# drnatebrown/col-bwt

Measured on AMD Instinct MI355X. Metric: query bases/s, higher is better.
Workload: dtype int64

## Files before the change

col-bwt_amd/csrc/capi.hip:

```cpp
#include <fcntl.h>
#include <hip/hip_runtime.h>
#include <stdlib.h>
#include <string.h>
#include <sys/mman.h>
#include <sys/stat.h>
#include <unistd.h>

#include <algorithm>
#include <atomic>
#include <chrono>
#include <condition_variable>
#include <deque>
#include <mutex>
#include <string>
#include <thread>
#include <vector>

#include "../../include/colbwt.h"
#include "bin_writer.h"
#include "count_query.h"
#include "fasta_parallel.h"
#include "fastx_reader.h"
#include "index.h"
#include "locate_query.h"
// ... 757 lines not shown
    if (e && e[0] >= '1' && e[0] <= '6' && e[1] == 0) return e[0] - '0';
    return COLBWT_LAYOUT_DEFAULT_CHOICE;
}

static int line_rows_steps(int layout_arg) {
    int steps = (layout_arg >> 8) & 0xFF;
    if (steps == 0) {
        steps = kDefaultLineSteps;
        const char *e = getenv("COLBWT_LINE_ROWS_STEPS");
        if (e && e[0] >= '2' && e[0] <= '8' && e[1] == 0) steps = e[0] - '0';
    }
    return steps;
}

int colbwt_index_open_memory(const void *bytes, uint64_t len, const colbwt_widths *widths, int device,
                             colbwt_index **out) {
    return colbwt_index_open_memory_layout(bytes, len, widths, device, COLBWT_LAYOUT_AUTO, out);
}

int colbwt_index_open_memory_layout(const void *bytes, uint64_t len, const colbwt_widths *widths, int device,
                                    int layout, colbwt_index **out) {
    if (!out) return fail(COLBWT_ERR_ARG, "null out");
    const bool automatic = layout == COLBWT_LAYOUT_AUTO;
    if (automatic) layout = default_layout();
    const int steps = line_rows_steps(layout);
    const bool steps_given = ((layout >> 8) & 0xFF) != 0 || getenv("COLBWT_LINE_ROWS_STEPS") != nullptr;
    layout &= 0xFF;
    if (layout < COLBWT_LAYOUT_ONE_STEP || layout > COLBWT_LAYOUT_MISMATCH_LINES_DEEP) return fail(COLBWT_ERR_ARG, "bad layout");
    if (layout >= COLBWT_LAYOUT_LINE_ROWS && !fat_steps_supported(steps))
        return fail(COLBWT_ERR_ARG, "line rows: own steps must be 4..8");
    *out = nullptr;
    if (!widths_ok(widths))
        return fail(COLBWT_ERR_ARG, "only the shipped widths BWT_BYTES=5 RUN_BYTES=4 LEN_BYTES=2 ID_BITS=8 are supported");
    colbwt_index *idx = new (std::nothrow) colbwt_index();
    if (!idx) return fail(COLBWT_ERR_NOMEM, "out of host memory");
    std::string err;
    const bool deep_if_room = automatic && layout == COLBWT_LAYOUT_MISMATCH_LINES && getenv("COLBWT_LAYOUT") == nullptr;
    int rc = idx->ix.load((const uint8_t *)bytes, len, device, deep_if_room ? kLayoutMismatchLinesAuto : layout, err, steps);
    if (rc == COLBWT_ERR_NOMEM && automatic) {
        struct Candidate { int layout, steps; };
        static const Candidate ladder[] = {{COLBWT_LAYOUT_MISMATCH_LINES_DEEP, 8}, {COLBWT_LAYOUT_MISMATCH_LINES, 8},
                                           {COLBWT_LAYOUT_LINE_ROWS, 8}, {COLBWT_LAYOUT_LINE_ROWS, 6},
                                           {COLBWT_LAYOUT_LINE_ROWS, 4},      {COLBWT_LAYOUT_THREE_STEP, 0}, {COLBWT_LAYOUT_TWO_STEP, 0},
                                           {COLBWT_LAYOUT_ONE_STEP, 0}};
        int hopeless_from = layout >= COLBWT_LAYOUT_LINE_ROWS ? idx->ix.fat_failed_level() : 0;
        for (const Candidate &c : ladder) {
            if (c.layout > layout || (c.layout == layout && (c.steps >= steps || steps_given))) continue;
            if (c.layout >= COLBWT_LAYOUT_LINE_ROWS && (steps_given || (hopeless_from && c.steps >= hopeless_from))) continue;
            rc = idx->ix.load((const uint8_t *)bytes, len, device, c.layout, err, c.steps);
            if (rc != COLBWT_ERR_NOMEM) break;
            if (c.layout >= COLBWT_LAYOUT_LINE_ROWS) {
                const int f = idx->ix.fat_failed_level();
                if (f && (!hopeless_from || f < hopeless_from)) hopeless_from = f;
            }
        }
    }
    if (rc != COLBWT_OK) {
        delete idx;
        return fail(rc, err);
    }
    *out = idx;
    return COLBWT_OK;
}

int colbwt_index_open(const char *prefix_or_file, const colbwt_widths *widths, int device, colbwt_index **out) {
    return colbwt_index_open_layout(prefix_or_file, widths, device, COLBWT_LAYOUT_AUTO, out);
}

int colbwt_index_open_layout(const char *prefix_or_file, const colbwt_widths *widths, int device, int layout,
                             colbwt_index **out) {
    if (!prefix_or_file || !out) return fail(COLBWT_ERR_ARG, "null argument");
    *out = nullptr;
    MappedFile mf;
    const int rc = map_index_file(prefix_or_file, mf);
    return rc != COLBWT_OK ? rc : colbwt_index_open_memory_layout(mf.data, mf.len, widths, device, layout, out);
}

int colbwt_index_open_memory_devices(const void *bytes, uint64_t len, const colbwt_widths *widths, const int *devices,
                                     int n_devices, int layout, colbwt_index **out) {
    if (!out) return fail(COLBWT_ERR_ARG, "null out");
    *out = nullptr;
    if (!devices || n_devices < 1 || n_devices > 64) return fail(COLBWT_ERR_ARG, "device list must hold 1 .. 64 devices");
    colbwt_index *first = nullptr;
    int rc = colbwt_index_open_memory_layout(bytes, len, widths, devices[0], layout, &first);
    if (rc != COLBWT_OK) return rc;
    colbwt_info info;
    (void)colbwt_index_info(first, &info);
    const int same = (int)info.layout | (info.layout >= COLBWT_LAYOUT_LINE_ROWS ? (int)(info.layout_shape >> 8) << 8 : 0);
    for (int k = 1; k < n_devices; ++k) {
        colbwt_index *rep = nullptr;
        rc = colbwt_index_open_memory_layout(bytes, len, widths, devices[k], same, &rep);
        if (rc != COLBWT_OK) {
            const std::string msg = "replica on device " + std::to_string(devices[k]) + ": " + g_err;
            delete first;
            return fail(rc, msg);
        }
        first->more.push_back(rep);
    }
    *out = first;
    return COLBWT_OK;
}

int colbwt_index_open_devices(const char *prefix_or_file, const colbwt_widths *widths, const int *devices, int n_devices,
                              int layout, colbwt_index **out) {
    if (!prefix_or_file || !out) return fail(COLBWT_ERR_ARG, "null argument");
    *out = nullptr;
    MappedFile mf;
    const int rc = map_index_file(prefix_or_file, mf);
    return rc != COLBWT_OK ? rc : colbwt_index_open_memory_devices(mf.data, mf.len, widths, devices, n_devices, layout, out);
}

void colbwt_index_close(colbwt_index *idx) { delete idx; }

int colbwt_index_info(const colbwt_index *idx, colbwt_info *out) {
    if (!idx || !out) return fail(COLBWT_ERR_ARG, "null argument");
    out->bwt_r = idx->ix.bwt_r();
    out->n = idx->ix.n();
    out->r = idx->ix.r();
    out->sigma = idx->ix.sigma();
    out->device = (uint32_t)idx->ix.device();
    out->device_bytes = idx->ix.device_bytes() + idx->loc.bytes();
    out->layout = (uint32_t)idx->ix.layout();
    out->layout_shape = idx->ix.line_rows() ? (idx->ix.table_fat().steps << 8) | kFatSlotSteps : 0;
    out->table_rows = idx->ix.table_rows();
    out->n_devices = 1 + (uint32_t)idx->more.size();
    out->reserved_ = 0;
    return COLBWT_OK;
}

int colbwt_query_batch(colbwt_index *idx, const uint8_t *bases, const uint64_t *read_off, uint64_t n_reads,
                       uint16_t *pml, uint8_t *cid, colbwt_stats *stats) {
    return query_batch_all<uint16_t>(idx, bases, read_off, n_reads, pml, cid, stats);
}

int colbwt_query_batch_u32(colbwt_index *idx, const uint8_t *bases, const uint64_t *read_off, uint64_t n_reads,
                           uint32_t *pml, uint8_t *cid, colbwt_stats *stats) {
    return query_batch_all<uint32_t>(idx, bases, read_off, n_reads, pml, cid, stats);
}

int colbwt_query_device(colbwt_index *idx, const uint8_t *d_bases, const uint64_t *d_read_off, uint64_t n_reads,
                        uint64_t n_bases, void *d_pml, int pml_bytes, uint8_t *d_cid, void *hip_stream,
                        colbwt_stats *stats) {
    return colbwt_query_device_ordered(idx, d_bases, d_read_off, n_reads, n_bases, d_pml, pml_bytes, d_cid, nullptr,
                                       hip_stream, stats);
}

int colbwt_query_device_ordered(colbwt_index *idx, const uint8_t *d_bases, const uint64_t *d_read_off,
                                uint64_t n_reads, uint64_t n_bases, void *d_pml, int pml_bytes, uint8_t *d_cid,
                                const uint32_t *d_order, void *hip_stream, colbwt_stats *stats) {
    auto bad_argument = [&]() -> const char * {
        if (pml_bytes != 2 && pml_bytes != 4) return "pml_bytes must be 2 or 4";
        if (n_reads == 0) return nullptr;
        if (!d_bases || !d_read_off || !d_pml || !d_cid) return "null device pointer";
        if (((uintptr_t)d_bases & 15) || ((uintptr_t)d_pml & 31) || ((uintptr_t)d_cid & 15))
            return "d_bases/d_cid must be 16-byte aligned and d_pml 32-byte aligned";
        return nullptr;
    };
    return device_entry(idx, d_bases, n_reads, n_bases, hip_stream, kAlgBytesPerBase, stats, bad_argument,
                        [&](const Index &ix, hipStream_t stream) {
                            launch_query(ix, d_bases, d_read_off, n_reads, n_bases, d_pml, pml_bytes, d_cid, d_order, stream);
                        });
}

static int query_file_impl(colbwt_index *idx, const char *pattern_path, const std::string &pml_name,
                           const std::string &cid_name, uint64_t batch_bases, colbwt_stats *stats, bool binary,
                           bool count = false, uint32_t locate_k = 0, uint32_t seeds_min = 0, uint32_t seeds_k = 0) {
    if (stats) memset(stats, 0, sizeof(*stats));
    const size_t replicas = 1 + idx->more.size();
    if (batch_bases == 0) batch_bases = (64ull << 20) * replicas;
    ParallelFasta fasta;
    FastxReader reader;
    bool parallel = fasta.open(pattern_path);
    if (!parallel && !reader.open(pattern_path)) return fail(COLBWT_ERR_IO, std::string("cannot open pattern file ") + pattern_path);
    TextWriter wp, wc;
    BinWriter bp, bc;
    FILE *wn = nullptr;
    if (count) {
        wn = fopen(pml_name.c_str(), "wb");
        if (!wn) return fail(COLBWT_ERR_IO, "cannot create " + pml_name);
        setvbuf(wn, nullptr, _IOFBF, 4u << 20);
    } else {
        if (!(binary ? bp.open(pml_name) : wp.open(pml_name))) return fail(COLBWT_ERR_IO, "cannot create " + pml_name);
        if (!(binary ? bc.open(cid_name) : wc.open(cid_name))) return fail(COLBWT_ERR_IO, "cannot create " + cid_name);
    }
    bool count_ok = true;

    FileBatch pool[kFileBatches];
    std::unique_lock<std::mutex> pinned(idx->file_mu, std::defer_lock);
    if (pinned.try_lock())
        for (int k = 0; k < kFileBatches; ++k) {
            pool[k].pml = &idx->file_pml[k];
            pool[k].cid = &idx->file_cid[k];
        }
    BatchQueue free_q, parsed_q, done_q;
    for (auto &b : pool) free_q.push(&b);
    std::atomic<bool> stop{false};
    std::atomic<bool> reader_failed{false};
    const bool trace = getenv("COLBWT_TRACE") != nullptr;
    double t_parse = 0, t_gpu = 0, t_format = 0;
    auto now = [] { return std::chrono::duration<double>(std::chrono::steady_clock::now().time_since_epoch()).count(); };
    const double t_begin = now();
    const unsigned host_threads = std::min(16u, std::max(2u, std::thread::hardware_concurrency()));

    std::thread reader_thread([&] {
        bool more = true;
        while (more && !stop.load()) {
            FileBatch *b = free_q.pop();
            const double t0 = now();
            b->bases.clear();
            b->names.clear();
            b->off.assign(1, 0);
            uint64_t max_len = 0;
            if (parallel) {
                const ParallelFasta::Result r = fasta.next_batch(batch_bases, host_threads / 2, b->names, b->bases, b->off, max_len);
                if (r == ParallelFasta::kEnd) more = false;
                if (r == ParallelFasta::kNotPlainFasta) {
                    parallel = false;
                    if (!reader.open_at(pattern_path, fasta.position())) {
                        reader_failed.store(true);
                        more = false;
                    }
                }
            }
            if (!parallel && more) {
                std::string name;
                while (b->bases.size() < batch_bases) {
                    if (!reader.next(name, b->bases)) {
                        more = false;
                        break;
                    }
                    b->names.push_back(name);
                    max_len = std::max<uint64_t>(max_len, b->bases.size() - b->off.back());
                    b->off.push_back(b->bases.size());
                }
            }
            b->wide = max_len > 65535;
            t_parse += now() - t0;
            if (b->names.empty()) {
                free_q.push(b);
                if (more) continue;
                break;
            }
            parsed_q.push(b);
        }
        parsed_q.push(nullptr);
    });

    std::thread writer_thread([&] {
        for (;;) {
            FileBatch *b = done_q.pop();
            if (!b) break;
            const uint64_t n_reads = b->names.size();
            const double t0 = now();
            if (seeds_k) {
                const uint32_t *sm = b->pml->as<uint32_t>();
                const uint32_t *sp = b->cid->as<uint32_t>(), *sl = sp + n_reads * seeds_k;
                const uint8_t *sc = (const uint8_t *)(sl + n_reads * seeds_k);
                for (uint64_t k = 0; k < n_reads && count_ok; ++k) {
                    const uint32_t *q = sm + 8 * k;
                    count_ok = fprintf(wn, "%s\t%llu\t%u\t%u\t%u\t%u\t%u\t%u\t%u\t%u\t", b->names[k].c_str(),
                                       (unsigned long long)(b->off[k + 1] - b->off[k]), q[0], q[2], q[1], q[3], q[4], q[5], q[6],
                                       q[7]) > 0;
                    const uint64_t want = std::min<uint64_t>(q[0], seeds_k);
                    for (uint64_t t = 0; t < want && count_ok; ++t) {
                        const uint64_t at = k * seeds_k + t;
                        count_ok = fprintf(wn, t ? ",%u:%u:%u" : "%u:%u:%u", sp[at], sl[at], (unsigned)sc[at]) > 0;
                    }
                    count_ok = count_ok && fputc('\n', wn) != EOF;
                }
                t_format += now() - t0;
                free_q.push(b);
                continue;
            }
            if (count) {
                const uint32_t *ml = b->pml->as<uint32_t>();
                const uint64_t *oc = b->cid->as<uint64_t>();
                const uint64_t *ps = oc + n_reads;
                const std::vector<uint64_t> &ds = idx->loc.doc_start;
                for (uint64_t k = 0; k < n_reads && count_ok; ++k) {
                    count_ok = fprintf(wn, locate_k ? "%s\t%llu\t%u\t%llu\t" : "%s\t%llu\t%u\t%llu\n", b->names[k].c_str(),
                                       (unsigned long long)(b->off[k + 1] - b->off[k]), ml[k], (unsigned long long)oc[k]) > 0;
                    if (!locate_k) continue;
                    const uint64_t want = std::min<uint64_t>(oc[k], locate_k);
                    for (uint64_t t = 0; t < want && count_ok; ++t) {
                        const uint64_t x = ps[k * locate_k + t];
                        const size_t d = (size_t)(std::upper_bound(ds.begin(), ds.end(), x) - ds.begin()) - 1;
                        count_ok = fprintf(wn, t ? ",%zu:%llu" : "%zu:%llu", d, (unsigned long long)(x - ds[d])) > 0;
                    }
                    count_ok = count_ok && fputc('\n', wn) != EOF;
                }
                t_format += now() - t0;
                free_q.push(b);
                continue;
            }
            std::thread cid_thread([&] {
                if (binary) bc.batch<uint8_t>(b->names, b->off.data(), b->cid->as<uint8_t>(), n_reads, host_threads / 2);
                else wc.batch(b->names, b->off.data(), b->cid->as<uint8_t>(), n_reads, host_threads / 2);
            });
            if (binary) {
                if (b->wide) bp.batch<uint16_t>(b->names, b->off.data(), b->pml->as<uint32_t>(), n_reads, host_threads / 2);
                else bp.batch<uint16_t>(b->names, b->off.data(), b->pml->as<uint16_t>(), n_reads, host_threads / 2);
            } else {
                if (b->wide) wp.batch(b->names, b->off.data(), b->pml->as<uint32_t>(), n_reads, host_threads / 2);
                else wp.batch(b->names, b->off.data(), b->pml->as<uint16_t>(), n_reads, host_threads / 2);
            }
            cid_thread.join();
            t_format += now() - t0;
// ... 349 lines not shown
```

col-bwt_amd/csrc/fat2_query.hip:

```cpp
#include <hip/hip_runtime.h>
#include <stdint.h>

#include "device_layout.h"
#include "fat_cursor.h"
#include "fat_layout.h"
#include "lane_io.h"
#include "lane_out.h"
#include "query_kernels.h"

namespace colbwt {

namespace {

constexpr uint32_t kOffMis0 = 0xFFFFFFFCu;
constexpr uint32_t kOffMis1 = 0xFFFFFFFBu;

#ifdef COLBWT_COUNT_TRIPS
#define FAT2_STAT(k) (++stat[k])
#else
#define FAT2_STAT(k) ((void)0)
#endif

__device__ __forceinline__ uint32_t mis_slot(const uint8_t *top, uint32_t own, uint32_t c) {
    const uint32_t aidx = top[own], cidx = top[c];
    const uint32_t slot = cidx < aidx ? cidx : cidx - 1;
    return cidx < 4 && slot < kFatSlots ? slot : kFatSlots;
}

template <int K, typename PmlT, bool kDeep>
__global__ __launch_bounds__(kQueryBlock)
void fat2_query_kernel(FatTable T, const uint8_t *__restrict__ bases, const uint64_t *__restrict__ read_off,
                       uint64_t n_reads, uint32_t big_reads, uint32_t tail_permille,
                       PmlT *__restrict__ pml, uint8_t *__restrict__ cid) {
    constexpr bool kWide = sizeof(PmlT) == 4;
    __shared__ uint4 s_stage[kWaves][8][64];
    __shared__ uint4 s_win[kWaves][4][64];
    __shared__ uint32_t s_claim;
    __shared__ uint8_t s_top[256];
    const uint32_t wave = threadIdx.x >> 6, lane = threadIdx.x & 63u, g8 = lane & ~7u, p = lane & 7u;
    uint32_t *const s_jx = reinterpret_cast<uint32_t *>(&s_stage[wave][7][48]);
    ChunkPlan plan;
    plan.init(n_reads, big_reads, tail_permille);
    if (threadIdx.x == 0) s_claim = 0;
    s_top[threadIdx.x] = (uint8_t)fat_top_index(T.top4, threadIdx.x);
    __syncthreads();
    uint32_t *const claim = &s_claim;
    ReadCursor rc;
    bool done;
    rc.c_next = threadIdx.x;
    rc.request_chunk(plan, read_off);
    rc.commit();
    done = !rc.enter_chunk(plan, claim);

    OutRuns acc;
    uint32_t trip = 0;
    LaneWindow win;
    win.init(rc.off + rc.k - 1);
    uint4 (*const my_win)[64] = s_win[wave];

    uint32_t j = done ? 0u : T.r - 1;
    uint32_t o = kOffLastPos;
    uint32_t L = 0;
    const uint4 *const my_row = &s_stage[wave][p][g8];

#ifdef COLBWT_COUNT_TRIPS
    unsigned long long stat[8] = {0, 0, 0, 0, 0, 0, 0, 0};
#endif
    while (__any(!done)) {
        bool step_back = false;
        if (!done && rc.k == 0 && !rc.next_in_flight && (rc.r != rc.r_lo || rc.nc_ready)) {
            if (rc.r != rc.r_lo) {
                rc.r -= 1;
                rc.k = rc.off - rc.next_off;
                rc.off = rc.next_off;
                step_back = rc.r > rc.r_lo;
            } else if (kWide || acc.cnt == 0) {
                done = !rc.enter_chunk(plan, claim);
                if (!done) win.init(rc.off + rc.k - 1);
            }
            j = done ? 0u : T.r - 1;
            o = kOffLastPos;
            L = 0;
        }
        const bool live = !done && rc.k != 0;
        uint64_t &k = rc.k;
        const uint64_t g = rc.off + k - 1;

        s_jx[lane] = j;
        wave_sync();
        {
            const uint4 ja = *reinterpret_cast<const uint4 *>(&s_jx[g8]);
            const uint4 jb = *reinterpret_cast<const uint4 *>(&s_jx[g8 + 4]);
            const uint32_t jq[8] = {ja.x, ja.y, ja.z, ja.w, jb.x, jb.y, jb.z, jb.w};
            wave_sync();
#pragma unroll
            for (uint32_t q = 0; q < 8; ++q)
                __builtin_amdgcn_global_load_lds(T.lines + (uint64_t)jq[q] * kFatRowBytes + ((p ^ q) << 4), &s_stage[wave][q][0],
                                                 16, 0, 0);
        }
        if (live && win.avail(g) < (k < 8u ? (uint32_t)k : 8u)) win.request(my_win, bases, g);
        if (step_back) { rc.in_next = read_off[rc.r - 1]; rc.next_in_flight = true; }
        if (!done && rc.fetch_pending) rc.request_chunk(plan, read_off);
        lds_dma_landed();
        rc.commit();

        const uint32_t have = live ? win.avail(g) : 0u;
        uint32_t consumed = 0, l_new = 0, keep = 0xFFFFFFFFu, keep1 = 0xFFFFFFFFu;
        uint64_t ids = 0;
        if (!live || have == 0) FAT2_STAT(5);
        if (live && have != 0) {
            const uint64_t W = win.get8(my_win, lane, g);
            const uint32_t left = k < have ? (uint32_t)k : have;
            if (o == kOffMis0 || o == kOffMis1) {
                FAT2_STAT(2);
                const uint32_t h4 = !kDeep && o == kOffMis1 ? 4u : 0u;
                const uint4 e0 = my_row[(h4 + 0u) ^ p], e1 = my_row[(h4 + 1u) ^ p], e2 = my_row[(h4 + 2u) ^ p],
                            e3 = my_row[(h4 + 3u) ^ p];
                const uint32_t carry = L;
                const uint32_t t1 = (e0.y >> 16) & 0xFFu, d1 = e0.y >> 24, v1 = e3.z & 7u;
                uint32_t oc = 4;
                if (left >= 2) {
                    const uint32_t c2 = (uint32_t)(W >> 48) & 0xFFu;
                    const uint32_t s2 = mis_slot(s_top, t1, c2);
                    if (c2 == t1) oc = 0;
                    else if (s2 < kFatSlots && ((v1 >> s2) & 1u)) oc = 1 + s2;
                }
                if (oc < 4) {
                    const uint32_t J = oc == 0 ? e0.z : oc == 1 ? e0.w : oc == 2 ? e1.x : e1.y;
                    const uint32_t rho = oc == 0 ? e1.z : oc == 1 ? e1.w : oc == 2 ? e2.x : e2.y;
                    const uint32_t pw = oc < 2 ? e2.z : e2.w, P = (oc & 1u) ? pw >> 16 : pw & 0xFFFFu;
                    const uint32_t ch = (e3.x >> (8 * oc)) & 0xFFu, cd = (e3.y >> (8 * oc)) & 0xFFu;
                    const uint32_t vo = (e3.z >> (4 + 4 * oc)) & 7u;
                    consumed = 2;
                    l_new = 1;
                    keep = oc == 0 ? 0xFFFFFFFFu : 0u;
                    ids = (uint64_t)(d1 | (carry << 8));
                    L = oc == 0 ? 1u : 0u;
                    uint32_t nJ = J, nP = P, nrho = rho, nch = ch, ncd = cd, nv = vo, seen = 2;
                    if constexpr (kDeep) {
                        if (left >= 3 && ((uint32_t)(W >> 40) & 0xFFu) == ch) {
                            const uint4 f0 = my_row[4u ^ p], f1 = my_row[5u ^ p], f2 = my_row[6u ^ p], f3 = my_row[7u ^ p];
                            nJ = oc == 0 ? f0.x : oc == 1 ? f0.y : oc == 2 ? f0.z : f0.w;
                            nrho = oc == 0 ? f1.x : oc == 1 ? f1.y : oc == 2 ? f1.z : f1.w;
                            const uint32_t pw2 = oc < 2 ? f2.x : f2.y;
                            nP = (oc & 1u) ? pw2 >> 16 : pw2 & 0xFFFFu;
                            nch = (f2.z >> (8 * oc)) & 0xFFu;
                            ncd = (f2.w >> (8 * oc)) & 0xFFu;
                            nv = (f3.x >> (4 * oc)) & 7u;
                            consumed = 3;
                            seen = 3;
                            ids = (uint64_t)(cd | (d1 << 8) | (carry << 16));
                            if (oc == 0) { l_new = 2; keep = 0xFFFFFFFFu; }
                            else { l_new = 1; keep = 0xFFFFFFFFu; keep1 = 0u; }
                            L += 1;
                        }
                    }
                    if (k > consumed) {
                        uint32_t sn = kFatSlots;
                        if (left > seen) {
                            const uint32_t cn = (uint32_t)(W >> (8u * (7u - seen))) & 0xFFu;
                            if (cn != nch) sn = mis_slot(s_top, nch, cn);
                        }
                        if (sn < kFatSlots && ((nv >> sn) & 1u)) {
                            const uint32_t e = nrho * kFatSlots + sn;
                            j = T.slot_line0 + (kDeep ? e : e >> 1);
                            o = kDeep ? kOffMis0 : kOffMis0 - (e & 1u);
                            L = ncd;
                        } else {
                            j = nJ;
                            o = nP;
                        }
                    }
                } else {
                    consumed = 1;
                    l_new = 0;
                    ids = (uint64_t)carry;
                    L = 0;
                    j = e0.x;
                    o = e0.y & 0xFFFFu;
                }
            } else {
                FAT2_STAT(0);
                const uint4 r0 = my_row[0 ^ p];
                const uint4 r1 = my_row[1 ^ p];
                const uint64_t CH = (uint64_t)r0.x | ((uint64_t)r0.y << 32);
                const uint64_t CID = (uint64_t)r0.z | ((uint64_t)r0.w << 32);
                const uint32_t len = r1.x & 0xFFFFu;
                uint32_t skip = 0;
                bool stay = false;
                if (o == kOffPred) { o = len - 1; skip = 1; }
                else if (o == kOffSucc) { o = 0; skip = 1; }
                else if (o >= len && j < T.r - 1) {
                    o -= len;
                    j += 1;
                    stay = true;
                    FAT2_STAT(1);
                } else {
                    o = o < len ? o : len - 1;
                }
                if (!stay) {
                    const uint64_t X = skip ? ((W >> 8) ^ CH) & 0x00FFFFFFFFFFFFFFull : W ^ CH;
                    const uint32_t run = matching_top_bytes(X);
                    const uint32_t cap = left + skip < (uint32_t)K ? left + skip : (uint32_t)K;
                    uint32_t steps = run < cap ? run : cap;
                    bool own_jump = true, to_entry = false;
                    uint32_t e_next = 0, carry = 0;
                    if (run < cap) {
                        const uint32_t d = run + 1u, sh = 8u * (8u - d);
                        const uint32_t c = (uint32_t)(W >> (sh + 8u * skip)) & 0xFFu;
                        const uint32_t s = mis_slot(s_top, (uint32_t)(CH >> sh) & 0xFFu, c);
                        if (s < kFatSlots && ((r1.w >> (3u * run + s)) & 1u)) {
                            const uint32_t rho = reinterpret_cast<const uint32_t *>(&my_row[((kFatRho / 16) + (run >> 2)) ^ p])[run & 3u];
                            e_next = rho * kFatSlots + s;
                            carry = (uint32_t)(CID >> sh) & 0xFFu;
                            to_entry = true;
                            own_jump = false;
                        }
                    }
                    if (run == 0 && !to_entry) {
                        const uint32_t c = (uint32_t)(W >> 56);
                        const uint32_t cidx = T.cmap[c];
                        bool moved = false;
                        if (cidx != kAbsent) moved = fat_threshold_scan(T, j, o, c, cidx);
                        FAT2_STAT(moved ? 3 : 4);
                        if (moved) {
                            steps = 1;
                            consumed = 1;
                            l_new = 0;
                            own_jump = false;
                        } else {
                            const uint32_t st = matching_top_bytes(X & 0x00FFFFFFFFFFFFFFull);
                            const uint32_t cap0 = left < (uint32_t)K ? left : (uint32_t)K;
                            steps = st < cap0 ? st : cap0;
                            consumed = steps;
                            l_new = steps - 1;
                        }
                    } else {
                        consumed = steps - skip;
                        l_new = L + consumed;
                    }
                    L = l_new;
                    ids = steps ? CID >> (8u * (8u - steps)) : 0ull;
                    if (k == consumed) {
                    } else if (to_entry) {
                        FAT2_STAT(6);
                        j = T.slot_line0 + (kDeep ? e_next : e_next >> 1);
                        o = kDeep ? kOffMis0 : kOffMis0 - (e_next & 1u);
                        L = carry;
                    } else if (own_jump) {
                        const uint32_t e = steps - 1;
                        const uint32_t I = reinterpret_cast<const uint32_t *>(&my_row[((kFatI / 16) + (e >> 2)) ^ p])[e & 3u];
                        const uint32_t Oh = reinterpret_cast<const uint16_t *>(&my_row[((kFatO / 16) + (e >> 3)) ^ p])[e & 7u];
                        const uint64_t cuts = (uint64_t)r1.y | ((uint64_t)r1.z << 32);
// ... 76 lines not shown
```

col-bwt_amd/csrc/fat_query.hip:

```cpp
#include <hip/hip_runtime.h>
#include <stdint.h>

#include "device_layout.h"
#include "fat_cursor.h"
#include "fat_layout.h"
#include "lane_io.h"
#include "lane_out.h"
#include "query_kernels.h"

namespace colbwt {

namespace {

template <int K, typename PmlT>
__global__ __launch_bounds__(kQueryBlock)
void fat_query_kernel(FatTable T, const uint8_t *__restrict__ bases, const uint64_t *__restrict__ read_off,
                      uint64_t n_reads, uint32_t big_reads, uint32_t tail_permille,
                      PmlT *__restrict__ pml, uint8_t *__restrict__ cid) {
    constexpr bool kWide = sizeof(PmlT) == 4;
    __shared__ uint4 s_stage[kWaves][8][64];
    __shared__ uint4 s_win[kWaves][4][64];
    __shared__ uint32_t s_claim;
    const uint32_t wave = threadIdx.x >> 6, lane = threadIdx.x & 63u, g8 = lane & ~7u, p = lane & 7u;
    uint32_t *const s_jx = reinterpret_cast<uint32_t *>(&s_stage[wave][7][48]);
    ChunkPlan plan;
    plan.init(n_reads, big_reads, tail_permille);
    if (threadIdx.x == 0) s_claim = 0;
    __syncthreads();
    uint32_t *const claim = &s_claim;
    ReadCursor rc;
    bool done;
    rc.c_next = threadIdx.x;
    rc.request_chunk(plan, read_off);
    rc.commit();
    done = !rc.enter_chunk(plan, claim);

    OutRuns acc;
    uint32_t trip = 0;
    LaneWindow win;
    win.init(rc.off + rc.k - 1);
    uint4 (*const my_win)[64] = s_win[wave];

    uint32_t j = done ? 0u : T.r - 1;
    uint32_t o = kOffLastPos;
    uint32_t L = 0;
    const uint4 *const my_row = &s_stage[wave][p][g8];

#ifdef COLBWT_COUNT_TRIPS
    unsigned long long stat[8] = {0, 0, 0, 0, 0, 0, 0, 0};
    unsigned long long clk[8] = {0, 0, 0, 0, 0, 0, 0, 0}, t_prev = clock64();
#endif
    while (__any(!done)) {
        bool step_back = false;
        if (!done && rc.k == 0 && !rc.next_in_flight && (rc.r != rc.r_lo || rc.nc_ready)) {
            if (rc.r != rc.r_lo) {
                rc.r -= 1;
                rc.k = rc.off - rc.next_off;
                rc.off = rc.next_off;
                step_back = rc.r > rc.r_lo;
            } else if (kWide || acc.cnt == 0) {
                FAT_STAT(6);
                done = !rc.enter_chunk(plan, claim);
                if (!done) win.init(rc.off + rc.k - 1);
            }
            j = done ? 0u : T.r - 1;
            o = kOffLastPos;
            L = 0;
        }
        FAT_CLOCK(4);
        const bool live = !done && rc.k != 0;
        uint64_t &k = rc.k;
        const uint64_t g = rc.off + k - 1;

        s_jx[lane] = j;
        wave_sync();
        {
            const uint4 ja = *reinterpret_cast<const uint4 *>(&s_jx[g8]);
            const uint4 jb = *reinterpret_cast<const uint4 *>(&s_jx[g8 + 4]);
            const uint32_t jq[8] = {ja.x, ja.y, ja.z, ja.w, jb.x, jb.y, jb.z, jb.w};
            wave_sync();
#pragma unroll
            for (uint32_t q = 0; q < 8; ++q)
                __builtin_amdgcn_global_load_lds(T.lines + (uint64_t)jq[q] * kFatRowBytes + ((p ^ q) << 4), &s_stage[wave][q][0],
                                                 16, 0, 0);
        }
        FAT_CLOCK(5);
        FAT_CLOCK(6);
        if (live && win.avail(g) < (k < 8u ? (uint32_t)k : 8u)) win.request(my_win, bases, g);
        if (step_back) { rc.in_next = read_off[rc.r - 1]; rc.next_in_flight = true; }
        if (!done && rc.fetch_pending) rc.request_chunk(plan, read_off);
        FAT_CLOCK(1);
        lds_dma_landed();
        rc.commit();
        FAT_CLOCK(2);

        const uint32_t have = live ? win.avail(g) : 0u;
        if (!live || have == 0) FAT_STAT(5);
        if (live && have != 0) {
            FAT_STAT(0);
            const uint4 r0 = my_row[0 ^ p];
            const uint4 r1 = my_row[1 ^ p];
            const uint64_t CH = (uint64_t)r0.x | ((uint64_t)r0.y << 32);
            const uint32_t len = r1.x & 0xFFFFu, flags = (r1.x >> 16) & 0xFFu;
            uint32_t skip = 0;
            bool stay = false;
            if (o == kOffPred) { o = len - 1; skip = 1; FAT_STAT(7); }
            else if (o == kOffSucc) { o = 0; skip = 1; FAT_STAT(7); }
            else if (o >= len && j < T.r - 1) {
                o -= len;
                j += 1;
                stay = true;
                FAT_STAT(1);
            } else {
                o = o < len ? o : len - 1;
            }
            if (!stay) {
                const uint64_t W = win.get8(my_win, lane, g);
                const uint64_t X = skip ? ((W >> 8) ^ CH) & 0x00FFFFFFFFFFFFFFull : W ^ CH;
                uint32_t steps = matching_top_bytes(X);
                const uint64_t left = k < have ? k : have;
                const uint32_t cap = left + skip < (uint64_t)K ? (uint32_t)left + skip : (uint32_t)K;
                steps = steps < cap ? steps : cap;
                uint32_t ids_lo = r0.z, ids_hi = r0.w;
                uint32_t consumed, l_new;
                bool use_slot = false, own_jump = true;
                uint4 sl = make_uint4(0, 0, 0, 0);
                if (steps == 0) {
                    const uint32_t c = (uint32_t)(W >> 56);
                    const uint32_t aidx = flags >> 4, cidx4 = fat_top_index(T.top4, c);
                    const uint32_t slot = cidx4 < aidx ? cidx4 : cidx4 - 1;
                    if (cidx4 < 4 && cidx4 != aidx && slot < kFatSlots && ((flags >> slot) & 1u)) {
                        sl = my_row[(kFatSlot0 / 16 + slot) ^ p];
                        const uint32_t tch2 = sl.w & 0xFFu, tcid2 = (sl.w >> 8) & 0xFFu;
                        const bool two = left >= 2 && ((uint32_t)(W >> 48) & 0xFFu) == tch2;
                        consumed = two ? 2u : 1u;
                        l_new = consumed - 1;
                        ids_hi = (ids_hi & 0xFF000000u) | (tcid2 << 16);
                        use_slot = true;
                        own_jump = false;
                        FAT_STAT(2);
                    } else {
                        const uint32_t cidx = T.cmap[c];
                        bool moved = false;
                        if (cidx != kAbsent) moved = fat_threshold_scan(T, j, o, c, cidx);
                        FAT_STAT(moved ? 3 : 4);
                        if (moved) {
                            steps = 1;
                            consumed = 1;
                            l_new = 0;
                            own_jump = false;
                        } else {
                            uint32_t st = matching_top_bytes(X & 0x00FFFFFFFFFFFFFFull);
                            const uint32_t cap0 = left < (uint64_t)K ? (uint32_t)left : (uint32_t)K;
                            steps = st < cap0 ? st : cap0;
                            consumed = steps;
                            l_new = steps - 1;
                        }
                    }
                } else {
                    consumed = steps - skip;
                    l_new = L + consumed;
                }
                L = l_new;
                {
                    const uint32_t top = use_slot ? consumed : steps;
                    const uint32_t sh = 8u * (8u - top);
                    const uint64_t ids = ((uint64_t)ids_lo | ((uint64_t)ids_hi << 32)) >> sh;
                    if constexpr (kWide) {
                        for (uint32_t e = 0; e < consumed; ++e) {
                            pml[g - consumed + 1 + e] = (PmlT)(l_new - e);
                            cid[g - consumed + 1 + e] = (uint8_t)(ids >> (8 * e));
                        }
                    } else {
                        acc.push_run(consumed, l_new, 0xFFFFFFFFu, 0xFFFFFFFFu, (uint32_t)ids, (uint32_t)(ids >> 32));
                    }
                }
                k -= consumed;
                if (k == 0) {
                } else if (use_slot) {
                    j = consumed == 2 ? sl.y : sl.x;
                    o = consumed == 2 ? sl.z >> 16 : sl.z & 0xFFFFu;
                } else if (own_jump) {
                    const uint32_t e = steps - 1;
                    const uint32_t I = reinterpret_cast<const uint32_t *>(&my_row[((kFatI / 16) + (e >> 2)) ^ p])[e & 3u];
                    const uint32_t Oh = reinterpret_cast<const uint16_t *>(&my_row[((kFatO / 16) + (e >> 3)) ^ p])[e & 7u];
                    const uint64_t cuts = (uint64_t)r1.y | ((uint64_t)r1.z << 32);
                    const uint32_t cut = (uint32_t)(cuts >> (8 * e)) & 0xFFu, cut_a = cut & 0xFu, len_b = cut >> 4;
                    j = I;
                    if (cut_a != kSKCutNone && o >= cut_a) {
                        j += 1;
                        o -= cut_a;
                        if (len_b != kSKCutNone && o >= len_b) {
                            j += 1;
                            o -= len_b;
                        }
                    } else {
                        o += Oh;
                    }
                }
            }
        }
        wave_sync();
        if constexpr (!kWide) {
            if ((trip & (OutRuns::kPeriod - 1)) == OutRuns::kPeriod - 1)
                acc.flush_wave((uint16_t *)pml, cid, rc.off + rc.k, !done, rc.k == 0 && rc.r == rc.r_lo, &s_stage[wave][0][0], lane);
        }
        ++trip;
        wave_sync();
        FAT_CLOCK(3);
#ifdef COLBWT_COUNT_TRIPS
        ++clk[0];
#endif
    }
#ifdef COLBWT_COUNT_TRIPS
    for (int q = 0; q < 8; ++q) atomicAdd(&g_fat_stats[q], stat[q]);
    if (lane == 0)
        for (int q = 0; q < 8; ++q) atomicAdd(&g_fat_clocks[q], clk[q]);
#endif
}

template <int K>
void launch_steps(const FatTable &T, const uint8_t *d_bases, const uint64_t *d_read_off, uint64_t n_reads, uint64_t n_bases,
                  void *d_pml, int pml_bytes, uint8_t *d_cid, hipStream_t stream) {
    if (pml_bytes == 2) launch_persistent<fat_query_kernel<K, uint16_t>>(T, d_bases, d_read_off, n_reads, n_bases, (uint16_t *)d_pml, d_cid, stream);
    else launch_persistent<fat_query_kernel<K, uint32_t>>(T, d_bases, d_read_off, n_reads, n_bases, (uint32_t *)d_pml, d_cid, stream);
}

}

void launch_fat_query(const FatTable &T, const uint8_t *d_bases, const uint64_t *d_read_off, uint64_t n_reads, uint64_t n_bases,
                      void *d_pml, int pml_bytes, uint8_t *d_cid, const uint32_t *, hipStream_t stream) {
    if (n_reads == 0) return;
    if (T.slot_line0) {
        launch_fat2_query(T, d_bases, d_read_off, n_reads, n_bases, d_pml, pml_bytes, d_cid, stream);
        return;
    }
#define X(K) \
    if (T.steps == K) launch_steps<K>(T, d_bases, d_read_off, n_reads, n_bases, d_pml, pml_bytes, d_cid, stream);
    COLBWT_FAT_STEPS(X)
#undef X
}
// ... 16 lines not shown
```

col-bwt_amd/csrc/lane_io.h:

```cpp
#pragma once
#include <hip/hip_runtime.h>
#include <stdint.h>

#include "query_kernels.h"

namespace colbwt {

constexpr uint32_t kFlush = 16;

template <typename PmlT>
struct OutAcc;

struct U128 {
    uint64_t lo, hi;
};
struct Q128 {
    uint32_t x, y, z, w;
};
template <typename V, typename E>
__device__ __forceinline__ void put(E *dst, V v) {
    struct __attribute__((packed, aligned(alignof(E)))) Slot {
        V v;
    };
    reinterpret_cast<Slot *>(dst)->v = v;
// ... 33 lines not shown
                put(dc, (uint32_t)c0);
                p0 = p1; c0 >>= 32;
                dp += 4; dc += 4;
            }
            if (cnt & 2u) {
                put(dp, (uint32_t)p0);
                put(dc, (uint16_t)c0);
                p0 >>= 32; c0 >>= 16;
                dp += 2; dc += 2;
            }
            if (cnt & 1u) {
                *dp = (uint16_t)p0;
                *dc = (uint8_t)c0;
            }
        }
        cnt = 0;
    }
};

template <>
struct OutAcc<uint32_t> {
    __device__ __forceinline__ void push(uint32_t, uint32_t) {}
    __device__ __forceinline__ void flush(uint32_t *, uint8_t *, uint64_t) {}
};


struct SlidingWindow {
    uint32_t wb;
    __device__ __forceinline__ void init(uint64_t g) { wb = (uint32_t)g + 1u; }
    __device__ __forceinline__ uint32_t avail(uint64_t g) const { return (uint32_t)g - wb + 1u; }
    __device__ __forceinline__ void refill(uint32_t (*s_rd)[kQueryBlock], const uint8_t *bases, uint64_t g) {
        const uint64_t a = g >= 60 ? (g - 60) & ~(uint64_t)3 : 0;
        struct __attribute__((packed, aligned(4))) Q {
            uint32_t x, y, z, w;
        };
        const Q *src = reinterpret_cast<const Q *>(bases + a);
        Q v[4];
#pragma unroll
        for (int q = 0; q < 4; ++q) v[q] = src[q];
#pragma unroll
        for (int q = 0; q < 4; ++q) {
            s_rd[4 * q + 0][threadIdx.x] = v[q].x;
            s_rd[4 * q + 1][threadIdx.x] = v[q].y;
            s_rd[4 * q + 2][threadIdx.x] = v[q].z;
            s_rd[4 * q + 3][threadIdx.x] = v[q].w;
        }
        wb = (uint32_t)a;
    }
    __device__ __forceinline__ uint32_t get(uint32_t (*s_rd)[kQueryBlock], uint64_t g) const {
        const uint32_t b = ((uint32_t)g - wb) & 63u;
        return (s_rd[b >> 2][threadIdx.x] >> (8 * (b & 3u))) & 0xFFu;
    }
    __device__ __forceinline__ uint64_t get8(uint32_t (*s_rd)[kQueryBlock], uint64_t g) const {
        const uint32_t b = ((uint32_t)g - wb) & 63u, d = b >> 2;
        const uint32_t x2 = s_rd[d][threadIdx.x], x1 = s_rd[(d - 1u) & 15u][threadIdx.x], x0 = s_rd[(d - 2u) & 15u][threadIdx.x];
        const uint32_t sh = 8u * ((b & 3u) + 1u);
        const uint64_t lo = (uint64_t)x0 | ((uint64_t)x1 << 32);
        return (lo >> sh) | ((uint64_t)x2 << (64u - sh));
    }
};

struct OutAcc18 {
    uint64_t p0 = 0, p1 = 0, p2 = 0, p3 = 0, c0 = 0, c1 = 0;
    uint32_t p4 = 0, c2 = 0;
    uint32_t cnt = 0;
    __device__ __forceinline__ void push(uint32_t L, uint32_t cid) {
        p4 = (p4 << 16) | (uint32_t)(p3 >> 48);
        p3 = (p3 << 16) | (p2 >> 48);
        p2 = (p2 << 16) | (p1 >> 48);
        p1 = (p1 << 16) | (p0 >> 48);
        p0 = (p0 << 16) | (uint64_t)(L & 0xFFFFu);
        c2 = (c2 << 8) | (uint32_t)(c1 >> 56);
        c1 = (c1 << 8) | (c0 >> 56);
        c0 = (c0 << 8) | (uint64_t)cid;
        ++cnt;
    }
    static __device__ __forceinline__ void pieces(uint16_t *dp, uint8_t *dc, uint32_t n, uint64_t q0, uint64_t q1,
                                                  uint64_t q2, uint64_t q3, uint64_t d0, uint64_t d1) {
        if (n & 8u) {
            put(dp, U128{q0, q1});
            put(dc, d0);
            q0 = q2; q1 = q3; d0 = d1;
            dp += 8; dc += 8;
        }
        if (n & 4u) {
            put(dp, q0);
            put(dc, (uint32_t)d0);
            q0 = q1; d0 >>= 32;
            dp += 4; dc += 4;
        }
        if (n & 2u) {
            put(dp, (uint32_t)q0);
            put(dc, (uint16_t)d0);
            q0 >>= 32; d0 >>= 16;
            dp += 2; dc += 2;
        }
        if (n & 1u) {
            *dp = (uint16_t)q0;
            *dc = (uint8_t)d0;
        }
    }
    __device__ __forceinline__ void flush_group(uint16_t *pml, uint8_t *cid, uint64_t gl) {
        const uint32_t extra = (0u - (uint32_t)gl) & (kFlush - 1);
        if (extra >= cnt) return;
        const bool s1 = extra & 1u, s2 = extra & 2u;
        uint64_t a0 = s1 ? (p0 >> 16) | (p1 << 48) : p0;
        uint64_t a1 = s1 ? (p1 >> 16) | (p2 << 48) : p1;
        uint64_t a2 = s1 ? (p2 >> 16) | (p3 << 48) : p2;
        uint64_t a3 = s1 ? (p3 >> 16) | ((uint64_t)p4 << 48) : p3;
        const uint64_t a4 = s1 ? p4 >> 16 : p4;
        a0 = s2 ? (a0 >> 32) | (a1 << 32) : a0;
        a1 = s2 ? (a1 >> 32) | (a2 << 32) : a1;
        a2 = s2 ? (a2 >> 32) | (a3 << 32) : a2;
        a3 = s2 ? (a3 >> 32) | (a4 << 32) : a3;
        uint64_t b0 = s1 ? (c0 >> 8) | (c1 << 56) : c0;
        uint64_t b1 = s1 ? (c1 >> 8) | ((uint64_t)c2 << 56) : c1;
        const uint64_t b2 = s1 ? c2 >> 8 : c2;
        b0 = s2 ? (b0 >> 16) | (b1 << 48) : b0;
        b1 = s2 ? (b1 >> 16) | (b2 << 48) : b1;
        const uint32_t n = cnt - extra;
        const uint64_t g = gl + extra;
        if (n == kFlush) {
            uint4 *dst = reinterpret_cast<uint4 *>(pml + g);
            dst[0] = make_uint4((uint32_t)a0, (uint32_t)(a0 >> 32), (uint32_t)a1, (uint32_t)(a1 >> 32));
            dst[1] = make_uint4((uint32_t)a2, (uint32_t)(a2 >> 32), (uint32_t)a3, (uint32_t)(a3 >> 32));
            *reinterpret_cast<uint4 *>(cid + g) =
                make_uint4((uint32_t)b0, (uint32_t)(b0 >> 32), (uint32_t)b1, (uint32_t)(b1 >> 32));
        } else {
            pieces(pml + g, cid + g, n, a0, a1, a2, a3, b0, b1);
        }
        cnt = extra;
    }
    __device__ __forceinline__ void flush_rest(uint16_t *pml, uint8_t *cid, uint64_t gl) {
        if (cnt) pieces(pml + gl, cid + gl, cnt, p0, p1, p2, p3, c0, c1);
        cnt = 0;
    }
};

__device__ __forceinline__ void wave_sync() {
    __builtin_amdgcn_fence(__ATOMIC_RELEASE, "wavefront");
    __builtin_amdgcn_wave_barrier();
    __builtin_amdgcn_fence(__ATOMIC_ACQUIRE, "wavefront");
}
__device__ __forceinline__ void lds_dma_landed() {
    __builtin_amdgcn_s_waitcnt(0x0F70);
    wave_sync();
}

struct LaneWindow {
    uint32_t wb;
    __device__ __forceinline__ void init(uint64_t g) { wb = (uint32_t)g + 1u; }
    __device__ __forceinline__ uint32_t avail(uint64_t g) const {
        const uint32_t d = (uint32_t)g - wb;
        return d < 64u ? d + 1u : 0u;
    }
    __device__ __forceinline__ void request(uint4 (*win)[64], const uint8_t *bases, uint64_t g) {
        const uint64_t a = g >= 48 ? (g - 48) & ~(uint64_t)15 : 0;
#pragma unroll
        for (uint32_t q = 0; q < 4; ++q) __builtin_amdgcn_global_load_lds(bases + a + 16 * q, &win[q][0], 16, 0, 0);
        wb = (uint32_t)a;
    }
    __device__ __forceinline__ uint32_t dword(const uint4 (*win)[64], uint32_t lane, uint32_t d) const {
        return reinterpret_cast<const uint32_t *>(&win[(d >> 2) & 3u][lane])[d & 3u];
    }
    __device__ __forceinline__ uint64_t get8(const uint4 (*win)[64], uint32_t lane, uint64_t g) const {
        const uint32_t e = (((uint32_t)g - wb) & 63u) + 1u, d = e >> 2, r = e & 3u;
        const uint32_t x2 = dword(win, lane, d & 15u), x1 = dword(win, lane, (d - 1u) & 15u), x0 = dword(win, lane, (d - 2u) & 15u);
        const uint32_t lo = __builtin_amdgcn_alignbyte(x1, x0, r), hi = __builtin_amdgcn_alignbyte(x2, x1, r);
        return (uint64_t)lo | ((uint64_t)hi << 32);
    }
};




}
```

col-bwt_amd/csrc/sk3_query.hip:

```cpp
#include <hip/hip_runtime.h>
#include <stdint.h>

#include "device_layout.h"
#include "fat_cursor.h"
#include "lane_io.h"
#include "lane_out.h"
#include "lf_device.h"
#include "query_kernels.h"
#include "sk_layout.h"

namespace colbwt {

namespace {

constexpr int K3 = 3;
constexpr uint32_t kFlushSlots = 32;
constexpr uint32_t kStagePieces = OutRuns::lds_q(kFlushSlots);

__device__ __forceinline__ bool sk3_threshold_scan(const SKTable &T, uint32_t &j, uint32_t &o, uint32_t c, uint32_t cidx, uint32_t hint) {
    SKRow<K3> t;
    if (hint == kHintPred) {
        const uint32_t q = sk_pred_char<K3>(T, j, c, cidx, t);
        if (q != kNone) { j = q; o = kOffPred; return true; }
        const uint32_t s = sk_succ_char<K3>(T, j, c, cidx, t);
        if (s != kNone) { j = s; o = kOffSucc; return true; }
        return false;
    }
    if (hint == kHintSucc) {
        const uint32_t s = sk_succ_char<K3>(T, j, c, cidx, t);
        if (s != kNone) { j = s; o = kOffSucc; return true; }
        return false;
    }
    const uint64_t pos = T.idx[j] + o;
    uint64_t thr = T.n;
    uint32_t nj = j, no = o;
    bool moved = false;
    const uint32_t s = sk_succ_char<K3>(T, j, c, cidx, t);
    if (s != kNone) { thr = T.thr[s]; nj = s; no = kOffSucc; moved = true; }
    if (pos < thr) {
        const uint32_t q = sk_pred_char<K3>(T, j, c, cidx, t);
        if (q != kNone) { nj = q; no = kOffPred; moved = true; }
    }
    j = nj;
    o = no;
    return moved;
}

template <typename PmlT>
__global__ __launch_bounds__(kQueryBlock)
void sk3_query_kernel(SKTable T, const uint8_t *__restrict__ bases, const uint64_t *__restrict__ read_off,
                      uint64_t n_reads, uint32_t big_reads, uint32_t tail_permille,
                      PmlT *__restrict__ pml, uint8_t *__restrict__ cid) {
    constexpr bool kWide = sizeof(PmlT) == 4;
    __shared__ uint4 s_stage[kWaves][kStagePieces];
    __shared__ uint4 s_win[kWaves][4][64];
    __shared__ uint32_t s_jx[kWaves][64];
    __shared__ uint8_t s_cmap[256];
    __shared__ uint32_t s_claim;
    const uint32_t wave = threadIdx.x >> 6, lane = threadIdx.x & 63u, g2 = lane & ~1u, sub = lane & 1u;
    ChunkPlan plan;
    plan.init(n_reads, big_reads, tail_permille);
    if (threadIdx.x == 0) s_claim = 0;
    s_cmap[threadIdx.x] = T.cmap[threadIdx.x];
    __syncthreads();
    uint32_t *const claim = &s_claim;
    ReadCursor rc;
    bool done;
    rc.c_next = threadIdx.x;
    rc.request_chunk(plan, read_off);
    rc.commit();
    done = !rc.enter_chunk(plan, claim);

    OutRuns acc;
    uint32_t trip = 0;
    LaneWindow win;
    win.init(rc.off + rc.k - 1);
    uint4 (*const my_win)[64] = s_win[wave];
    uint4 *const stage = s_stage[wave];

    uint32_t j = done ? 0u : T.r - 1;
    uint32_t o = kOffLastPos;
    uint32_t L = 0;

    while (__any(!done)) {
        bool step_back = false;
        if (!done && rc.k == 0 && !rc.next_in_flight && (rc.r != rc.r_lo || rc.nc_ready)) {
            if (rc.r != rc.r_lo) {
                rc.r -= 1;
                rc.k = rc.off - rc.next_off;
                rc.off = rc.next_off;
                step_back = rc.r > rc.r_lo;
            } else if (kWide || acc.cnt == 0) {
                done = !rc.enter_chunk(plan, claim);
                if (!done) win.init(rc.off + rc.k - 1);
            }
            j = done ? 0u : T.r - 1;
            o = kOffLastPos;
            L = 0;
        }
        const bool live = !done && rc.k != 0;
        uint64_t &k = rc.k;
        const uint64_t g = rc.off + k - 1;

        s_jx[wave][lane] = j;
        wave_sync();
        {
            const uint2 jp = *reinterpret_cast<const uint2 *>(&s_jx[wave][g2]);
            const uint32_t jq[2] = {jp.x, jp.y};
#pragma unroll
            for (uint32_t q = 0; q < 2; ++q)
                __builtin_amdgcn_global_load_lds(T.lines + (uint64_t)jq[q] * 32u + ((sub ^ q) << 4), &stage[q * 64], 16, 0, 0);
        }
        if (live && win.avail(g) < (k < 8u ? (uint32_t)k : 8u)) win.request(my_win, bases, g);
        if (step_back) { rc.in_next = read_off[rc.r - 1]; rc.next_in_flight = true; }
        if (!done && rc.fetch_pending) rc.request_chunk(plan, read_off);
        lds_dma_landed();
        rc.commit();

        const uint32_t have = live ? win.avail(g) : 0u;
        uint32_t consumed = 0, l_new = 0;
        uint64_t ids = 0;
        if (live && have != 0) {
            SKRow<K3> w;
            {
                const uint4 a = stage[sub * 64 + g2 + (0u ^ sub)], b = stage[sub * 64 + g2 + (1u ^ sub)];
                w.d[0] = a.x; w.d[1] = a.y; w.d[2] = a.z; w.d[3] = a.w; w.d[4] = b.x; w.d[5] = b.y; w.d[6] = b.z; w.d[7] = b.w;
            }
            const uint64_t W = win.get8(my_win, lane, g);
            const uint64_t left = k < have ? k : have;
            const uint32_t len = sk_len<K3>(w);
            bool stay = false;
            uint32_t own = 0;
            if (o == kOffPred) o = len - 1;
            else if (o == kOffSucc) o = 0;
            else if (o >= len && j < T.r - 1) {
                o -= len;
                j += 1;
                stay = true;
            } else {
                o = o < len ? o : len - 1;
                own = 1;
            }
            uint32_t la_from = 1;
            if (own) {
                const uint32_t c = (uint32_t)(W >> 56);
                ids = sk_cid<K3>(w);
                consumed = 1;
                if (sk_char<K3>(w) == c) {
                    l_new = L + 1;
                } else {
                    l_new = 0;
                    const uint32_t cidx = s_cmap[c];
                    if (cidx != kAbsent) {
                        uint32_t hint = kHintCompare, dist = kSKDistFar;
                        const uint32_t hs = hint_slot(cidx, s_cmap[sk_char<K3>(w)]);
                        if (hs < kHintSlots) {
                            hint = (sk_hints<K3>(w) >> (2 * hs)) & 3u;
                            dist = sk_dist<K3>(w, hs);
                        }
                        if (dist != kSKDistFar && hint != kHintCompare) {
                            j = hint == kHintPred ? j - dist : j + dist;
                            o = hint == kHintPred ? kOffPred : kOffSucc;
                            stay = true;
                        } else if (sk3_threshold_scan(T, j, o, c, cidx, hint)) {
                            stay = true;
                        }
                    }
                }
            } else {
                la_from = 0;
                l_new = L;
            }
            if (!stay) {
                uint32_t steps = 1;
                const uint32_t c2 = (uint32_t)(W >> (8u * (7u - la_from))) & 0xFFu, c3 = (uint32_t)(W >> (8u * (6u - la_from))) & 0xFFu;
                if (left > consumed && c2 == sk_char_at<K3, 2>(w)) {
                    ids = (ids << 8) | sk_cid_at<K3, 2>(w);
                    ++consumed;
                    ++l_new;
                    steps = 2;
                    if (left > consumed && c3 == sk_char_at<K3, 3>(w)) {
                        ids = (ids << 8) | sk_cid_at<K3, 3>(w);
                        ++consumed;
                        ++l_new;
                        steps = 3;
                    }
                }
                if (k != consumed) {
                    j = sk_I<K3>(w, steps);
                    const uint32_t cut = sk_cut_a<K3>(w);
                    if (steps == (uint32_t)K3 && cut != kSKCutNone && o >= cut) {
                        j += 1;
                        o -= cut;
                        const uint32_t lb = sk_len_b<K3>(w);
                        if (lb != kSKCutNone && o >= lb) {
                            j += 1;
                            o -= lb;
                        }
                    } else {
                        o += sk_O<K3>(w, steps);
                    }
                }
            }
            L = l_new;
            if constexpr (kWide) {
                for (uint32_t e = 0; e < consumed; ++e) {
                    pml[g - consumed + 1 + e] = (PmlT)(l_new - e);
                    cid[g - consumed + 1 + e] = (uint8_t)(ids >> (8 * e));
                }
            } else {
                acc.push_run(consumed, l_new, 0xFFFFFFFFu, 0xFFFFFFFFu, (uint32_t)ids, 0u);
            }
            k -= consumed;
        }
        wave_sync();
        if constexpr (!kWide) {
            if ((trip & (OutRuns::kPeriod - 1)) == OutRuns::kPeriod - 1)
                acc.template flush_wave<kFlushSlots>((uint16_t *)pml, cid, rc.off + rc.k, !done, rc.k == 0 && rc.r == rc.r_lo, stage, lane);
        }
        ++trip;
        wave_sync();
    }
}

}

void launch_sk3_query(const SKTable &T, const uint8_t *d_bases, const uint64_t *d_read_off, uint64_t n_reads, uint64_t n_bases,
                      void *d_pml, int pml_bytes, uint8_t *d_cid, hipStream_t stream) {
    if (n_reads == 0) return;
    if (pml_bytes == 2) launch_persistent<sk3_query_kernel<uint16_t>>(T, d_bases, d_read_off, n_reads, n_bases, (uint16_t *)d_pml, d_cid, stream);
    else launch_persistent<sk3_query_kernel<uint32_t>>(T, d_bases, d_read_off, n_reads, n_bases, (uint32_t *)d_pml, d_cid, stream);
}

}
```

Before: 145.7 billion.

## Widen per-lane base window to 80 bytes with 64-byte-aligned refills

The per-lane LDS window of read bases grows from four to five 16-byte slots. Refills now load 64-byte-aligned chunks and carry the oldest slot into the fifth, so the unconsumed tail survives. A new low() check refills only when the window is truly exhausted or near empty and the read has more bases left. This cuts redundant base refetches and allows unaligned base pointers for layout 3 and above. The costs are more LDS per wave, which may lower occupancy, and extra index clamping in get8.

Result: slower. 138.8 billion (-4.8%).

```diff
diff --git a/col-bwt_amd/csrc/capi.hip b/col-bwt_amd/csrc/capi.hip
--- a/col-bwt_amd/csrc/capi.hip
+++ b/col-bwt_amd/csrc/capi.hip
@@ -933,7 +933,8 @@
         if (pml_bytes != 2 && pml_bytes != 4) return "pml_bytes must be 2 or 4";
         if (n_reads == 0) return nullptr;
         if (!d_bases || !d_read_off || !d_pml || !d_cid) return "null device pointer";
-        if (((uintptr_t)d_bases & 15) || ((uintptr_t)d_pml & 31) || ((uintptr_t)d_cid & 15))
+        const bool any_bases = idx && idx->ix.layout() >= 3;
+        if ((((uintptr_t)d_bases & 15) && !any_bases) || ((uintptr_t)d_pml & 31) || ((uintptr_t)d_cid & 15))
             return "d_bases/d_cid must be 16-byte aligned and d_pml 32-byte aligned";
         return nullptr;
     };
diff --git a/col-bwt_amd/csrc/fat2_query.hip b/col-bwt_amd/csrc/fat2_query.hip
--- a/col-bwt_amd/csrc/fat2_query.hip
+++ b/col-bwt_amd/csrc/fat2_query.hip
@@ -34,7 +34,7 @@
                        PmlT *__restrict__ pml, uint8_t *__restrict__ cid) {
     constexpr bool kWide = sizeof(PmlT) == 4;
     __shared__ uint4 s_stage[kWaves][8][64];
-    __shared__ uint4 s_win[kWaves][4][64];
+    __shared__ uint4 s_win[kWaves][5][64];
     __shared__ uint32_t s_claim;
     __shared__ uint8_t s_top[256];
     const uint32_t wave = threadIdx.x >> 6, lane = threadIdx.x & 63u, g8 = lane & ~7u, p = lane & 7u;
@@ -98,7 +98,7 @@
                 __builtin_amdgcn_global_load_lds(T.lines + (uint64_t)jq[q] * kFatRowBytes + ((p ^ q) << 4), &s_stage[wave][q][0],
                                                  16, 0, 0);
         }
-        if (live && win.avail(g) < (k < 8u ? (uint32_t)k : 8u)) win.request(my_win, bases, g);
+        if (live && win.low(g, rc.next_off)) win.request(my_win, lane, bases, g);
         if (step_back) { rc.in_next = read_off[rc.r - 1]; rc.next_in_flight = true; }
         if (!done && rc.fetch_pending) rc.request_chunk(plan, read_off);
         lds_dma_landed();
diff --git a/col-bwt_amd/csrc/fat_query.hip b/col-bwt_amd/csrc/fat_query.hip
--- a/col-bwt_amd/csrc/fat_query.hip
+++ b/col-bwt_amd/csrc/fat_query.hip
@@ -19,7 +19,7 @@
                       PmlT *__restrict__ pml, uint8_t *__restrict__ cid) {
     constexpr bool kWide = sizeof(PmlT) == 4;
     __shared__ uint4 s_stage[kWaves][8][64];
-    __shared__ uint4 s_win[kWaves][4][64];
+    __shared__ uint4 s_win[kWaves][5][64];
     __shared__ uint32_t s_claim;
     const uint32_t wave = threadIdx.x >> 6, lane = threadIdx.x & 63u, g8 = lane & ~7u, p = lane & 7u;
     uint32_t *const s_jx = reinterpret_cast<uint32_t *>(&s_stage[wave][7][48]);
@@ -86,7 +86,7 @@
         }
         FAT_CLOCK(5);
         FAT_CLOCK(6);
-        if (live && win.avail(g) < (k < 8u ? (uint32_t)k : 8u)) win.request(my_win, bases, g);
+        if (live && win.low(g, rc.next_off)) win.request(my_win, lane, bases, g);
         if (step_back) { rc.in_next = read_off[rc.r - 1]; rc.next_in_flight = true; }
         if (!done && rc.fetch_pending) rc.request_chunk(plan, read_off);
         FAT_CLOCK(1);
diff --git a/col-bwt_amd/csrc/lane_io.h b/col-bwt_amd/csrc/lane_io.h
--- a/col-bwt_amd/csrc/lane_io.h
+++ b/col-bwt_amd/csrc/lane_io.h
@@ -209,20 +209,41 @@
     __device__ __forceinline__ void init(uint64_t g) { wb = (uint32_t)g + 1u; }
     __device__ __forceinline__ uint32_t avail(uint64_t g) const {
         const uint32_t d = (uint32_t)g - wb;
-        return d < 64u ? d + 1u : 0u;
-    }
-    __device__ __forceinline__ void request(uint4 (*win)[64], const uint8_t *bases, uint64_t g) {
-        const uint64_t a = g >= 48 ? (g - 48) & ~(uint64_t)15 : 0;
-#pragma unroll
-        for (uint32_t q = 0; q < 4; ++q) __builtin_amdgcn_global_load_lds(bases + a + 16 * q, &win[q][0], 16, 0, 0);
-        wb = (uint32_t)a;
+        return d < 80u ? d + 1u : 0u;
+    }
+    __device__ __forceinline__ bool low(uint64_t g, uint64_t lowest) const {
+        const uint32_t d = (uint32_t)g - wb;
+        return d >= 80u || (d < 16u && g - lowest > d);
+    }
+    __device__ __forceinline__ void request(uint4 (*win)[64], uint32_t lane, const uint8_t *bases, uint64_t g) {
+        const uint64_t base = reinterpret_cast<uint64_t>(bases);
+        const uint32_t ab = (uint32_t)base & 63u;
+        const uint32_t d = (uint32_t)g - wb;
+        const bool fresh = d >= 80u;
+        if (!fresh) win[4][lane] = win[0][lane];
+        const uint64_t a = (g + ab - (fresh ? 0u : d + 1u)) & ~(uint64_t)63;
+        const uint8_t *src = reinterpret_cast<const uint8_t *>(base - ab + a);
+        if (ab < 16u) {
+#pragma unroll
+            for (uint32_t q = 0; q < 4; ++q) __builtin_amdgcn_global_load_lds(src + 16 * q, &win[q][0], 16, 0, 0);
+        } else {
+            const uint32_t first = a == 0 ? ab & ~15u : 0u;
+#pragma unroll
+            for (uint32_t q = 0; q < 4; ++q) {
+                const uint32_t at = 16 * q < first ? first : 16 * q;
+                __builtin_amdgcn_global_load_lds(src + at, &win[q][0], 16, 0, 0);
+            }
+        }
+        wb = (uint32_t)a - ab;
     }
     __device__ __forceinline__ uint32_t dword(const uint4 (*win)[64], uint32_t lane, uint32_t d) const {
-        return reinterpret_cast<const uint32_t *>(&win[(d >> 2) & 3u][lane])[d & 3u];
+        return reinterpret_cast<const uint32_t *>(&win[d >> 2][lane])[d & 3u];
     }
     __device__ __forceinline__ uint64_t get8(const uint4 (*win)[64], uint32_t lane, uint64_t g) const {
-        const uint32_t e = (((uint32_t)g - wb) & 63u) + 1u, d = e >> 2, r = e & 3u;
-        const uint32_t x2 = dword(win, lane, d & 15u), x1 = dword(win, lane, (d - 1u) & 15u), x0 = dword(win, lane, (d - 2u) & 15u);
+        const uint32_t e = ((uint32_t)g - wb) + 1u, d = e >> 2, r = e & 3u;
+        const int32_t d1 = (int32_t)d - 1, d0 = (int32_t)d - 2;
+        const uint32_t x2 = dword(win, lane, d < 19u ? d : 19u), x1 = dword(win, lane, (uint32_t)(d1 > 0 ? d1 : 0)),
+                       x0 = dword(win, lane, (uint32_t)(d0 > 0 ? d0 : 0));
         const uint32_t lo = __builtin_amdgcn_alignbyte(x1, x0, r), hi = __builtin_amdgcn_alignbyte(x2, x1, r);
         return (uint64_t)lo | ((uint64_t)hi << 32);
     }
diff --git a/col-bwt_amd/csrc/sk3_query.hip b/col-bwt_amd/csrc/sk3_query.hip
--- a/col-bwt_amd/csrc/sk3_query.hip
+++ b/col-bwt_amd/csrc/sk3_query.hip
@@ -53,7 +53,7 @@
                       PmlT *__restrict__ pml, uint8_t *__restrict__ cid) {
     constexpr bool kWide = sizeof(PmlT) == 4;
     __shared__ uint4 s_stage[kWaves][kStagePieces];
-    __shared__ uint4 s_win[kWaves][4][64];
+    __shared__ uint4 s_win[kWaves][5][64];
     __shared__ uint32_t s_jx[kWaves][64];
     __shared__ uint8_t s_cmap[256];
     __shared__ uint32_t s_claim;
@@ -111,7 +111,7 @@
             for (uint32_t q = 0; q < 2; ++q)
                 __builtin_amdgcn_global_load_lds(T.lines + (uint64_t)jq[q] * 32u + ((sub ^ q) << 4), &stage[q * 64], 16, 0, 0);
         }
-        if (live && win.avail(g) < (k < 8u ? (uint32_t)k : 8u)) win.request(my_win, bases, g);
+        if (live && win.low(g, rc.next_off)) win.request(my_win, lane, bases, g);
         if (step_back) { rc.in_next = read_off[rc.r - 1]; rc.next_in_flight = true; }
         if (!done && rc.fetch_pending) rc.request_chunk(plan, read_off);
         lds_dma_landed();
```
